# YaqiangCao/cLoops

Hardware: AMD Instinct MI355X
Metric: PETs clustered/sec (whole node) + wall-clock for mode-3 eps x minPts sweep (higher is better)
Workload: dtype int32; 1 GPU; synthetic-200M-23chr-mode3 (BASELINE.json configs[3]); variant=cDBSCAN2, pets=200000000, chromosomes=23, chained_cut=True, final_cut=3871, candidate_loops=3651369, parallelism=23 chromosomes LPT-sharded over 1 GPU(s)

## Files before the change

### cloops_amd/csrc/cl_chrom.h

```cpp
#pragma once
#include "cl_common.h"
#include "cl_table.h"
#include "cl_prim.h"
#include "cl_textout.h"

#define BIGTPB 1024
#define AGG_H 512
__device__ __forceinline__ int agg_slot(int* keys, int key)
{
    unsigned h = ((unsigned)key * 2654435761u) >> 23;
    for (int probe = 0; probe < 24; ++probe) {
        const int old = atomicCAS(&keys[h], -1, key);
        if (old == -1 || old == key) return (int)h;
        h = (h + 1) & (AGG_H - 1);
    }
    return -1;
}
#define FLAT_PER 4
struct Stats { int amin, amax, vmin, vmax, xmin, xmax, ymin, ymax; };
__device__ __forceinline__ int je_minus(const int* __restrict__ cstart, int j) { return cstart[j + 1] - cstart[j]; }
static inline int bits_for(unsigned v) { int b = 0; while (v) { ++b; v >>= 1; } return b; }


#define CL_FINE_KMAX 8
#define K7_BLOCKS 2048
#define K7_STEP_BLOCKS 256
#define K7_STEP_THREADS 1024
#define K7_LOGBINS 3840
__device__ __forceinline__ int k7_logbin(unsigned d)
{
    const int e = 31 - __clz((int)d);
    const unsigned m = e >= 7 ? ((d >> (e - 7)) & 127u) : ((d << (7 - e)) & 127u);
    return e * 128 + (int)m;
}
#define K7_FINE 2048
#define K7_XSHIFT 11.0
#define CAND_BLOCK 2048

struct K7Src {
    int sorted;
    int n; int M; int v0;
    const int* dM;
    const int* X; const int* Y; const int* labels;
    const int* sv; const int* slab;
    const int* dh;
};

struct K7Part { double sx[2]; double sxx[2]; long long n_all[2]; long long n_pos[2]; };

enum { HDR_K = 0, HDR_ERR = 1, HDR_M = 2, HDR_NCLUSTERS = 3, HDR_MAXLABEL = 4, HDR_TRUNC = 5, HDR_LABELLED = 6, HDR_WORDS = 16 };
enum { HDR_ERR_STRIP = 4 , HDR_ERR_COUNT = 8  };

struct RunRequest {
    int variant = CL_VARIANT_CDBSCAN1, eps = 0, minPts = 0, cut = 0;
    int32_t* labels_out = nullptr;
    int2* pairs_out = nullptr;
    long long pairs_cap = 0;
    void* mask_out = nullptr;
    long long mask_cap = 0;
    int step = -1;
    long long fine_lo = -1;
    int wx = 0, wy = 0;
};

struct cl_chrom {
    long long tmp_n = -1;
    DevBuf arena;
    int device = 0;
    hipStream_t stream = nullptr;
    bool own_stream = false;
    int64_t n = 0;
    int *d_x = nullptr, *d_y = nullptr;
    bool own_xy = false;
    Stats st{};
    DevBuf keys_in, keys_out, vals_in, vals_out, sort_tmp, scan_tmp;
    DevBuf qb_key, qb_val;
    int qindex_layout = -1;
    struct Fine {
        DevBuf q, sp, row, strip;
        DevBuf dead;
        int w = 0;
        int valid_w = 0, layout = -1;
        GridParams g;
        void invalidate() { valid_w = 0; layout = -1; }
    } fine;
    int sort_index_mode = 0;
    long long n_sorts = 0;
    DevBuf sv, sa, strip, cnt, parent, root, head, headidx, cellfirst, compkey, ncore, bsize, owner, state;
    DevBuf flag, rankscan, ulist, lo, hi, recs, counters, chainflag, chainhead, usize, b_cstart, b_ckey, b_nb, b_cx, b_cy, tile_s0;
    int* h_pinned = nullptr;
    struct StripPlan { int layout, eps, maxlen; };
    std::vector<StripPlan> plans;
    struct Held {
        int32_t* labels_out = nullptr;
        struct Extra {
            void* dst = nullptr;
            long long cap = 0;
            size_t fixed = 0; int per = 0;
            bool copy_empty = false;
            const char* refusal = nullptr;
        } extra;
        int n_strips = 0;
        bool band_timed = false;
        long long n_queried = 0;
        bool exported = false;
        bool step_valid = false;
        bool host_written = false;
        bool wait_done = false;
        long long fine_lo = -1;
        bool rows_valid = false;
        bool sorted_src = false;
        const int* k7_sv = nullptr;
        const int* k7_lcnt = nullptr;
        int k7_v0 = 0;
    };
    struct Run {
        u32* srow = nullptr;
        int *sv = nullptr, *sa = nullptr, *strip = nullptr, *tile = nullptr;
        int* cnt = nullptr;
        WordSrc ws{};
        int init_nclr = 0;
        int level = 0;
        const int* dM = nullptr;
        int m = 0;
        bool m_exact = false;
        bool rows = true;
        bool l4_make_base = false;
        bool l4_cut = false;
        bool l4_band = false;
        bool k2_make = false;
        const int* k_total = nullptr;
        bool hdr_packed = false;
        int kmax = 0;
        Held held;
    } run;
    struct Base {
        DevBuf q, sp, row, strip, tile, key;
        bool valid = false; int layout = -1, eps = 0;
        bool key_valid = false;
        int floor_q = 0;
        int rows = 0;
        long long pad_rows = -1;
        void invalidate() { valid = false; key_valid = false; floor_q = 0; }
    } base;
    bool sweep_planned = false;
    DevBuf sel_tmp;
    struct Counts {
        bool valid = false;
        bool cut_on_base = false;
        bool base_space = false;
        int layout = -1, eps = 0, thr = 0 , cap = 0;
        u32 tmask[4] = {0, 0, 0, 0};
        DevBuf cnt, pre, poff, dpre, D, blen;
        void invalidate() { valid = false; }
    } rc;
    bool reuse_counts = true;
    int count_floor = 0;
    u32 count_tmask[4] = {0, 0, 0, 0};
    DevBuf blk_tmp;
    DevBuf rootlist, cflag8;
    DevBuf l_mask, l_rank, l_blk, l_cstrip, l_wpos, l_wenc, l_dist, l_aux;
    DevBuf l_tab, l_fix;
    bool pairs_defer = false, pairs_copy_pending = false;
    bool fuse_chains = true;
    bool l_sup_dirty = false;
    GridParams dbg_g{}; int dbg_nm = 0;
    int traversal = 4;
    int last_k2_mode = 0;
    std::vector<long long> dcum;
    DevBuf dhist;
    long long n_neg = 0;
    bool reuse_layout = true;
    struct Slot {
        DevBuf labels, table;
        DevBuf slab;
        DevBuf pairs;
        DevBuf d_step;
        hipEvent_t ev_done = nullptr, ev_copied = nullptr;
        hipEvent_t ev[10]{};
        int* h_hdr = nullptr;
        char* h_step = nullptr;
        cl_box* h_boxes = nullptr;
        size_t h_boxes_cap = 0;
        bool pending = false;
        Held held;
    } slot[2];
    bool device_labels = true;
    bool export_table = true;
    struct Cand { DevBuf box, step, keep, out; long long n = 0, cap = 0; } cand;
    DevBuf hdr;
    DevBuf k7_cls, k7_parts;
    struct Kde {
        DevBuf ent, sorted, ctr, tmp, part;
        int run = -1;
        long long cap = 0, cnt[2] = {0, 0};
    } kde;
    struct Sig { DevBuf tx, ty, tmp, sorttmp, m, win, out; bool ready = false; int cut = 0; } sig;
    struct Fp { DevBuf small, keys, sorted, tmp, pairs; } fp;
    struct Anchor { DevBuf s, e, dir, mask, wsum; } an;
    struct Agg {
        DevBuf kin, vin, sx, sy, tmp, m, cx, cy, lkin, lkout, lvin, order, ltmp, sum, stats, mats;
        bool ready = false; int cut = 0, kept = 0;
    } ag;
    struct Track {
        DevBuf tcnt, toff, row, keys, sorted, tmp, ids, names;
        TextOut txt;
        struct State {
            bool built = false, ids = false;
            int kind = 0, la = 0, lb = 0, gbits = 0;
            long long cut = 0, ext = 0;
        } st;
    } tk;
    struct Cov {
        DevBuf kin, key, tmp, dcur, dprev, xr, flag, scan, ctr, start, end, depth, name;
// ... 279 lines not shown
```

### cloops_amd/csrc/cloops_hip.hip

```cpp
#include <map>
#include <mutex>
#include "cl_chrom.h"
#include "cl_band.h"

thread_local std::string g_err;



extern "C" const char* cl_last_error(void) { return g_err.c_str(); }
extern "C" int cl_version(void) { return CL_VERSION_NUM; }

extern "C" void* cl_host_alloc(int64_t bytes)
{
    void* p = nullptr;
    if (bytes <= 0) return nullptr;
    if (hipHostMalloc(&p, (size_t)bytes, hipHostMallocDefault) != hipSuccess) { fail(CL_ERR_HIP, "hipHostMalloc"); return nullptr; }
    return p;
}
extern "C" void cl_host_free(void* p) { if (p) (void)hipHostFree(p); }

static std::mutex g_pair_mu;
static std::map<hipStream_t, hipStream_t> g_copy_of;
extern "C" void* cl_stream_create(int device)
{
// ... 2786 lines not shown
__global__ void k_pack_header(int* __restrict__ hdr, const int* __restrict__ rankscan_total, const int* __restrict__ counters,
                              const int* __restrict__ d_M)
{
    if (threadIdx.x == 0 && blockIdx.x == 0) {
        hdr[HDR_K] = rankscan_total[0];
        hdr[HDR_ERR] = counters[CTR_OVERFLOW];
        hdr[HDR_M] = d_M[0];
        hdr[HDR_NCLUSTERS] = 0;
        hdr[HDR_MAXLABEL] = -1;
        hdr[HDR_TRUNC] = 0;
    }
}

__global__ void k_export_table(int* __restrict__ hdr, Table t, cl_box* __restrict__ host_rows, int cap)
{
    const int K = hdr[HDR_K];
    const bool store = cap >= 0;
    const int lim = store ? min(K, cap) : K;
    int nc = 0, ml = -1;
    for (int k = blockIdx.x * blockDim.x + threadIdx.x; k < lim; k += gridDim.x * blockDim.x) {
        if (store) {
            cl_box b = t.get(k);
            if (b.count > 0) { ++nc; ml = k; } else { b.min_x = b.max_x = b.min_y = b.max_y = 0; }
            host_rows[k] = b;
        } else if (t.count[k] > 0) { ++nc; ml = k; }
    }
    for (int o = 32; o > 0; o >>= 1) { nc += __shfl_down(nc, o); ml = max(ml, __shfl_down(ml, o)); }
    if ((threadIdx.x & 63) == 0) {
        if (nc) atomicAdd(&hdr[HDR_NCLUSTERS], nc);
        if (ml >= 0) atomicMax(&hdr[HDR_MAXLABEL], ml);
    }
    if (blockIdx.x == 0 && threadIdx.x == 0 && store && K > cap) hdr[HDR_TRUNC] = 1;
}

Table make_table_slot(cl_chrom* c, int slot)
{
    Table t;
    int* base = c->slot[slot].table.as<int>();
    const size_t stride = (size_t)c->n + 1;
    t.count = base; t.minx = base + stride; t.maxx = base + 2 * stride; t.miny = base + 3 * stride; t.maxy = base + 4 * stride;
    return t;
}
Table make_table(cl_chrom* c) { return make_table_slot(c, c->cur); }

const int* k7_hist_for(cl_chrom* c, int cut)
{
    return (cut > 0 && cut < DCUM_BINS && c->n_neg == 0 && !c->dcum.empty() && c->dhist.p) ? c->dhist.as<int>() : (const int*)nullptr;
}

K7Src k7_src(cl_chrom* c, const cl_chrom::Held& r, cl_chrom::Slot& sl, int cut, int M, const int* dM)
{
    K7Src s{};
    s.sorted = r.sorted_src ? (r.k7_lcnt ? 2 : 1) : 0; s.n = (int)c->n; s.M = M; s.v0 = r.k7_v0; s.dM = r.k7_lcnt ? r.k7_lcnt : dM;
    s.X = c->d_x; s.Y = c->d_y; s.labels = sl.labels.as<int>(); s.sv = r.k7_sv; s.slab = sl.slab.as<int>();
    s.dh = k7_hist_for(c, cut);
    return s;
}

int finish_enqueue(cl_chrom* c, const RunRequest& req, int n_strips, const int* d_M)
{
    const int n = (int)c->n;
    int32_t* const labels_out = req.labels_out;
    cl_chrom::Slot& sl = c->slot[c->cur];
    cl_chrom::Held& held = c->run.held;
    int* dh = c->hdr.as<int>() + HDR_WORDS * c->cur;
    if (sl.h_boxes_cap == 0 && c->export_table && req.step < 0) {
        const size_t cap = (size_t)n / 16 + 65536;
        HIP_TRY(hipHostMalloc((void**)&sl.h_boxes, cap * sizeof(cl_box), hipHostMallocDefault));
        sl.h_boxes_cap = cap;
    }
    if (!c->run.hdr_packed)
        hipLaunchKernelGGL(k_pack_header, dim3(1), dim3(64), 0, c->stream, dh, c->run.k_total ? c->run.k_total : c->rankscan.as<int>() + n, c->counters.as<int>(), d_M);
    const bool exported = c->export_table && req.step < 0;
    if (req.step < 0)
        hipLaunchKernelGGL(k_export_table, dim3(256), dim3(TPB), 0, c->stream, dh, make_table(c), sl.h_boxes,
                           exported ? (int)std::min<size_t>(sl.h_boxes_cap, 0x7fffffff) : -1);
    held.exported = exported;
    if (req.step >= 0) {
        int rc;
        if ((rc = c->k7_cls.ensure((size_t)n + 16))) return rc;
        const int kmax = std::max(1, std::min(c->run.kmax, n));
        if ((rc = ensure_cand_capacity(c, c->cand.n + kmax))) return rc;
        const size_t out_bytes = 16 + sizeof(K7Part) + K7_LOGBINS * 8 + K7_FINE * 8;
        if ((rc = sl.d_step.ensure(out_bytes + K7_BLOCKS * sizeof(K7Part)))) return rc;
        const int nb = nblocks(kmax, CAND_BLOCK);
        if ((rc = c->sel_tmp.ensure((size_t)nb * 12 + 64))) return rc;
        int* bcount = c->sel_tmp.as<int>();
        Table t = make_table(c);
        signed char* cls = c->k7_cls.as<signed char>();
        char* ds = (char*)sl.d_step.p;
        unsigned long long* lh = (unsigned long long*)(ds + 16 + sizeof(K7Part));
        hipLaunchKernelGGL(k_step_classify_count, dim3(nb), dim3(256), 0, c->stream, (const int*)dh, t, cls, bcount, nb,
                           lh, K7_LOGBINS + K7_FINE);
        hipLaunchKernelGGL(k_cand_append, dim3(nb), dim3(256), 0, c->stream, (const int*)dh, cls, t, (const int*)nullptr, (const int*)bcount,
                           (int)c->cand.n, req.step, (int)std::min<long long>(c->cand.cap, INT_MAX), c->cand.box.as<int4>(), c->cand.step.as<int>());
        K7Part* parts = (K7Part*)(ds + out_bytes);
        const K7Src src = k7_src(c, held, sl, req.cut, 0, d_M);
        int k7b = K7_STEP_BLOCKS;
#ifdef CLOOPS_DEVEL
        int k7t = K7_STEP_THREADS;
        { const char* e = getenv("CLOOPS_K7B"); if (e) k7b = std::max(1, std::min(atoi(e), K7_BLOCKS)); e = getenv("CLOOPS_K7T"); if (e) k7t = atoi(e); }
#else
        const int k7t = K7_STEP_THREADS;
#endif
        if (!SKIP(16)) hipLaunchKernelGGL(k7_summary, dim3(k7b), dim3(k7t), 0, c->stream, src, req.cut, cls, parts, lh,
                           (unsigned)req.fine_lo, req.fine_lo >= 0 ? lh + K7_LOGBINS : (unsigned long long*)nullptr);
        static_assert((16 + sizeof(K7Part)) % 8 == 0, "step output in 8-byte words");
// ... 383 lines not shown
                       pmax32, c->parent.as<int>());
    if (level == 0 && !SKIP(4)) hipLaunchKernelGGL(k_flatten, dim3(nblocks(nm, BIGTPB * FLAT_PER)), dim3(BIGTPB), 0, c->stream, g, strip, (const int*)nullptr, (const int*)c->chainflag.as<int>(),
           c->parent.as<int>(), srow, c->head.as<int>(), c->cellfirst.as<int>(),
           c->root.as<int>(), c->compkey.as<int>(), c->ncore.as<int>(), c->rootlist.as<int>(), counters);
    int* rootlist = c->rootlist.as<int>();
    ev_record(c, 4);
    int* clist = c->chainflag.as<int>();
    if (level >= 2) { if ((rc = lists_border(c, g, nm, L))) return rc; }
    else if (wide == 0) {
        const int nt_b = nblocks(std::max(1, c->run.m), 1024);
        if (!SKIP(1)) hipLaunchKernelGGL((k_border<1024, 128, TPB>), dim3(tile_grid(nt_b)), dim3(TPB), 0, c->stream, g, nt_b, sv, sa, strip, c->root.as<int>(),
                           c->compkey.as<int>(), c->ncore.as<int>(), srow, c->owner.as<int>(), c->bsize.as<int>(), c->usize.as<int>(), ws, clist, counters);
    } else
    TILE_LAUNCH_H((wide >= 2 && wide <= 4) ? 512 : (wide >= 5 ? 256 : 128), k_border, g, ntiles, sv, sa, strip, c->root.as<int>(), c->compkey.as<int>(),
                       c->ncore.as<int>(), srow, c->owner.as<int>(), c->bsize.as<int>(), c->usize.as<int>(), ws, clist, counters);
    if (variant == CL_VARIANT_CDBSCAN2) {
        const int rec_cap = n;
        hipLaunchKernelGGL(k_mark_uncertain_l, dim3(512), dim3(TPB), 0, c->stream, g, rootlist, c->ncore.as<int>(), c->bsize.as<int>(), c->state.as<int>(),
                           c->ulist.as<int>(), counters);
        if (level >= 2) { if ((rc = lists_emit_records(c, g, nm, L))) return rc; }
        else if (!SKIP(128)) hipLaunchKernelGGL(k_emit_records, dim3(2048), dim3(TPB), 0, c->stream, g, sv, sa, strip, c->root.as<int>(),
                           c->compkey.as<int>(), c->state.as<int>(), c->owner.as<int>(), c->recs.as<Rec>(), rec_cap, counters,
                           (const int*)clist, ws);
        hipLaunchKernelGGL(k_resolve_release, dim3(1), dim3(1024), 0, c->stream, minPts, c->ncore.as<int>(), c->usize.as<int>(), c->state.as<int>(),
                           c->ulist.as<int>(), c->recs.as<Rec>(), c->lo.as<int>(), c->hi.as<int>(), counters);
    }
    ev_record(c, 5);
    hipLaunchKernelGGL(k_rank_bits_l, dim3(512), dim3(TPB), 0, c->stream, g, rootlist, counters, c->compkey.as<int>(), c->state.as<int>(), c->flag.as<unsigned>(),
                       variant == CL_VARIANT_CDBSCAN2 ? (const Rec*)c->recs.as<Rec>() : (const Rec*)nullptr, c->owner.as<int>());
    const int nblkw = nblocks(nw, 1024);
    if ((rc = c->blk_tmp.ensure(((size_t)nblkw + 2) * 8))) return rc;
    int* wbsum = c->blk_tmp.as<int>();
    int* wboff = wbsum + nblkw + 1;
    hipLaunchKernelGGL(k_rank_scan, dim3(nblkw), dim3(256), 0, c->stream, nw, (const unsigned*)c->flag.as<unsigned>(), c->rankscan.as<int>(), wbsum, wboff,
                       counters + CTR_TICKET_B);
    c->run.k_total = wboff + nblkw;
    Table t = make_table(c);
    hipLaunchKernelGGL(k_root_labels_bits_l, dim3(512), dim3(TPB), 0, c->stream, g, rootlist, counters, c->compkey.as<int>(), c->ncore.as<int>(), c->bsize.as<int>(),
                       c->state.as<int>(), c->flag.as<unsigned>(), (const int*)c->rankscan.as<int>(), (const int*)wboff, c->chainhead.as<int>(), t, nblkw,
                       c->hdr.as<int>() + HDR_WORDS * c->cur, c->run.dM ? c->run.dM : (const int*)(strip + g.S));
    c->run.hdr_packed = true;
    if (level >= 3) {
        int* const labelled = c->hdr.as<int>() + HDR_WORDS * c->cur + HDR_LABELLED;
        if (req.pairs_out) {
            held.extra = {req.pairs_out, req.pairs_cap, 0, 8, false, "cl_cluster_pairs_async: the run labelled more PETs than capacity_pairs (n always suffices)"};
            if ((rc = c->slot[c->cur].pairs.ensure((size_t)std::max<long long>(req.pairs_cap, 1) * 8))) return rc;
        }
        if ((rc = lists_final(c, req, g, nm, L, rows, labelled))) return rc;
        if (req.mask_out) {
            held.extra = {req.mask_out, req.mask_cap, (size_t)((n + 63) / 64) * 8, 4, true, "cl_cluster_rowmask_async: the run labelled more PETs than capacity_labels (n always suffices)"};
            if ((rc = lists_rowmask(c, req, labelled))) return rc;
        }
        held.k7_lcnt = L.lcnt; held.k7_sv = c->l_dist.as<int>();
    } else {
        if (req.mask_out) return fail(CL_ERR_ARG, "cl_cluster_rowmask_async: this run did not take the list form");
        if (level == 2 && (rc = lists_scatter_owner(c, nm, L))) return rc;
        if (!SKIP(8)) hipLaunchKernelGGL(k_final_labels, dim3(nblocks(nm, BIGTPB * FINAL_CHUNKS)), dim3(BIGTPB), 0, c->stream, g, strip, sv, sa, srow,
                       level == 2 ? c->l_aux.as<int>() : c->owner.as<int>(),
                       c->chainhead.as<int>(), rows ? c->slot[c->cur].labels.as<int>() : (int*)nullptr, c->slot[c->cur].slab.as<int>(), t);
    }
    HIP_TRY(hipGetLastError());
    rc = finish_enqueue(c, req, g.S + 2, c->run.dM ? c->run.dM : strip + g.S);
    guard.armed = rc != CL_OK;
    return rc;
}


extern "C" int cl_get_boxes(cl_chrom* c, cl_box* boxes_out)
{
    if (!c) return fail(CL_ERR_ARG, "null chromosome handle");
    if (!c->have_result) return fail(CL_ERR_ARG, "cl_get_boxes: no clustering result available");
    const int K = c->last_K;
    if (K <= 0) return CL_OK;
    if (!boxes_out) return fail(CL_ERR_ARG, "boxes_out is null");
    if (c->last_slot >= 0 && !c->slot[c->last_slot].held.exported) return fail(CL_ERR_ARG, "cl_get_boxes: the run was made with the table export switched off");
    memcpy(boxes_out, c->slot[c->last_slot].h_boxes, (size_t)K * sizeof(cl_box));
    return CL_OK;
}

extern "C" int64_t cl_last_n_in(const cl_chrom* c)
{
    if (!c || !c->have_result || c->last_slot < 0) return 0;
    return c->slot[c->last_slot].h_hdr[HDR_M];
}

extern "C" const cl_box* cl_boxes_host(const cl_chrom* c)
{
    if (!c || !c->have_result || c->last_slot < 0 || c->last_K <= 0 || !c->slot[c->last_slot].held.exported) return nullptr;
    return c->slot[c->last_slot].h_boxes;
}
```

### cloops_amd/csrc/k_lists.hip

```cpp
#include "cl_chrom.h"

#ifdef CLOOPS_DEVEL
#define L_ABL(bit) (g.dbg2 & (bit))
#else
#define L_ABL(bit) 0
#endif
#ifdef CLOOPS_DEVEL
__device__ unsigned long long g_lstat[32];
__device__ __forceinline__ void lstat_add(int slot, int v)
{
    int t = v;
    for (int o = 32; o > 0; o >>= 1) t += __shfl_down(t, o);
    if ((threadIdx.x & 63) == 0 && t) atomicAdd(&g_lstat[slot], (unsigned long long)t);
}
extern "C" void cl_debug_lstats(unsigned long long* out)
{
    (void)hipDeviceSynchronize();
    (void)hipMemcpyFromSymbol(out, HIP_SYMBOL(g_lstat), sizeof(g_lstat));
    unsigned long long z[32] = {0};
    (void)hipMemcpyToSymbol(HIP_SYMBOL(g_lstat), z, sizeof(z));
}
#define LSTAT_ON (g.dbg2 & (1 << 30))
#define LSTAT(slot, v) do { if (LSTAT_ON) lstat_add((slot), (v)); } while (0)
#else
// ... 1566 lines not shown
            auto more = [&](int w, int q, int p) {
                return w == 0 ? ((p >= pbeg) & (q >= qlo)) : w == 1 ? ((p < pend) & (q <= qhi)) : w == 2 ? ((p < pbeg) & (q <= qhi)) : ((p < pend2) & (q <= qhi));
            };
            auto acc = [&](int w, int p) { return w == 2 ? p >= plo : (w == 3 ? p <= phi : true); };
            auto round = [&](int w, bool on, bool in, int2 p, int r) {
                const bool ok = on && in && more(w, p.x, p.y);
                const int rv = (ok && acc(w, p.y)) ? r : -1;
                unsigned pending = (unsigned)(__ballot(rv >= 0) >> gsh) & 0xffffu;
                while (__any(pending != 0u)) {
                    const int R = __shfl(rv, gsh + (pending ? __ffs((int)pending) - 1 : 0));
                    const unsigned same = (unsigned)(__ballot(pending != 0u && rv == R) >> gsh) & 0xffffu;
                    if (pending) { see(R); pending &= ~same; }
                }
                return on && ((unsigned)(__ballot(ok) >> gsh) & 0xffffu) == 0xffffu;
            };
            int2 p0[4]; int r0[4]; bool in0[4];
#pragma unroll
            for (int w = 0; w < 4; ++w) {
                const int j = w == 0 ? start[w] - gl : start[w] + gl;
                in0[w] = act && j >= 0 && j < C;
                p0[w] = in0[w] ? cpair[j] : make_int2(0, 0); r0[w] = in0[w] ? croot[j] : -1;
            }
#pragma unroll
            for (int w = 0; w < 4; ++w) {
                bool on = round(w, act, in0[w], p0[w], r0[w]);
                for (int rnd = 1; __any(on); ++rnd) {
                    const int j = w == 0 ? start[w] - gl - EG * rnd : start[w] + gl + EG * rnd;
                    const bool in = on && j >= 0 && j < C;
                    on = round(w, on, in, in ? cpair[j] : make_int2(0, 0), in ? croot[j] : -1);
                }
            }
            if (act && gl == 0) {
                if (overflow) atomicExch(&counters[CTR_OVERFLOW], 1);
                if (any_u) {
                    const int idx = atomicAdd(&counters[CTR_NREC], 1);
                    if (idx >= rec_cap) atomicExch(&counters[CTR_OVERFLOW], 2);
                    else {
                        Rec rec; rec.pt = h;
                        for (int q = 0; q < 4; ++q) rec.r[q] = rr[q];
                        recs[idx] = rec;
                    }
                }
            }
        }
    }
}

#ifndef LF_TPB
#define LF_TPB BIGTPB
#endif
#ifndef LF_CHUNKS
#define LF_CHUNKS 2
#endif
__global__ void __launch_bounds__(LF_TPB)
k_final_lists(GridParams g, const int* __restrict__ lcnt, const int2* __restrict__ cpair, const int* __restrict__ cpos,
              const int* __restrict__ croot, const int2* __restrict__ wpair, const int* __restrict__ wpos,
              const int* __restrict__ wowner, const int* __restrict__ rlabel, const u32* __restrict__ srow,
              int* __restrict__ labels, int* __restrict__ llab, int* __restrict__ ldist, Table t,
              int2* __restrict__ pairs , int pairs_cap,
              int* __restrict__ pair_count)
{
    __shared__ TableLds h;
    table_lds_init(h);
    const int C = lcnt[0], L = C + lcnt[1];
    int idx[LF_CHUNKS], own[LF_CHUNKS], lab[LF_CHUNKS], x[LF_CHUNKS], y[LF_CHUNKS], pos[LF_CHUNKS];
    int2 pr[LF_CHUNKS];
#pragma unroll
    for (int ch = 0; ch < LF_CHUNKS; ++ch) {
        idx[ch] = (blockIdx.x * LF_CHUNKS + ch) * LF_TPB + threadIdx.x;
        const int k = idx[ch];
        own[ch] = -1; pos[ch] = 0; pr[ch] = make_int2(0, 0);
        if (k < C) { own[ch] = croot[k]; pr[ch] = cpair[k]; pos[ch] = (labels || pairs) ? cpos[k] : 0; }
        else if (k < L) { own[ch] = owner_root(wowner[k - C]); pr[ch] = wpair[k - C]; pos[ch] = (labels || pairs) ? wpos[k - C] : 0; }
    }
#pragma unroll
    for (int ch = 0; ch < LF_CHUNKS; ++ch) lab[ch] = own[ch] >= 0 ? rlabel[own[ch]] : -1;
#pragma unroll
    for (int ch = 0; ch < LF_CHUNKS; ++ch) {
        const int k = idx[ch];
        x[ch] = 0; y[ch] = 0;
        if (k < L) {
            llab[k] = lab[ch];
            ldist[k] = pr[ch].x;
            if (lab[ch] >= 0) {
                if (labels) labels[srow[pos[ch]]] = lab[ch];
                const int spv = pr[ch].y;
                const int pp = ((spv >> g.rbits) + g.s0) * g.eps + (spv & (g.peps - 1)) + g.A0, qq = pr[ch].x + g.V0;
                const int a = g.swap ? qq : pp, v = g.swap ? pp : qq;
                x[ch] = (v - a) / 2; y[ch] = (v + a) / 2;
            }
        }
    }
    if (pairs) {
        __shared__ int l_pc[LF_CHUNKS * (LF_TPB / 64)];
        __shared__ int l_pbase;
        const int lane = threadIdx.x & 63, wv = threadIdx.x >> 6;
        unsigned long long bals[LF_CHUNKS];
#pragma unroll
        for (int ch = 0; ch < LF_CHUNKS; ++ch) {
            bals[ch] = __ballot(lab[ch] >= 0);
            if (lane == 0) l_pc[ch * (LF_TPB / 64) + wv] = __popcll(bals[ch]);
        }
        __syncthreads();
        if (threadIdx.x == 0) {
            int tot = 0;
            for (int k = 0; k < LF_CHUNKS * (LF_TPB / 64); ++k) { const int v = l_pc[k]; l_pc[k] = tot; tot += v; }
            l_pbase = tot ? atomicAdd(pair_count, tot) : 0;
        }
        __syncthreads();
#pragma unroll
        for (int ch = 0; ch < LF_CHUNKS; ++ch) {
            if (lab[ch] < 0) continue;
            const int at = l_pbase + l_pc[ch * (LF_TPB / 64) + wv] + lane_rank(bals[ch]);
            if (at < pairs_cap) pairs[at] = make_int2((int)srow[pos[ch]], lab[ch]);
        }
    }
    if (L_ABL(1 << 10)) return;
#pragma unroll
    for (int ch = 0; ch < LF_CHUNKS; ++ch) table_accumulate(t, h, lab[ch], x[ch], y[ch]);
    if (L_ABL(1 << 9)) return;
    table_flush(t, h);
}

struct ListBufs {
    unsigned long long *cmask, *wmask, *hmask;
    int *cgloc, *wgloc, *cgrank, *wgrank;
    int *bsum, *sup, *lcnt;
    int nsup2;
};
static int list_bufs(cl_chrom* c, const GridParams& g, int nm, ListBufs* b)
{
    const size_t n = (size_t)c->n;
    const size_t ngrp_cap = n / 64 + LG + 4;
    const size_t nblk_cap = n / LT + 4;
    int rc;
    if ((rc = c->l_mask.ensure(3 * ngrp_cap * 8)) || (rc = c->l_rank.ensure(4 * ngrp_cap * 4)) ||
        (rc = c->l_blk.ensure((2 * (nblk_cap + 1) + 2 * (nblk_cap / 16 + 4) + 16) * 4)) || (rc = c->l_cstrip.ensure(((size_t)g.S + 4) * 4)) ||
        (rc = c->l_wpos.ensure(n * 4)) || (rc = c->l_wenc.ensure(n * 4)) || (rc = c->l_dist.ensure(n * 4)) ||
        (c->traversal < 3 && (rc = c->l_aux.ensure(n * 4)))) return rc;
    b->cmask = c->l_mask.as<unsigned long long>(); b->wmask = b->cmask + ngrp_cap; b->hmask = b->wmask + ngrp_cap;
    b->cgloc = c->l_rank.as<int>(); b->wgloc = b->cgloc + ngrp_cap; b->cgrank = b->wgloc + ngrp_cap; b->wgrank = b->cgrank + ngrp_cap;
    const int nblk = nblocks(nm, LT);
    const size_t nsup_cap = nblk_cap / 16 + 4;
    if (c->l_blk.fresh) {
        HIP_TRY(hipMemsetAsync(c->l_blk.p, 0, c->l_blk.bytes, c->stream));
        c->l_blk.fresh = false;
    }
    b->lcnt = c->l_blk.as<int>();
    b->sup = b->lcnt + 8;
    b->bsum = b->sup + 2 * nsup_cap;
    b->nsup2 = 2 * ((nblk + 63) / 64 + 1);
    return CL_OK;
}

static void launch_classify(cl_chrom* c, const GridParams& g, int nblk, const ListBufs& b)
{
#define LA_ARGS g, (const int*)c->run.sv, (const int*)c->run.sa, (const int*)c->run.strip, c->run.ws, (const u32*)c->run.srow, b.cmask, b.wmask, b.hmask, b.cgloc, b.wgloc, b.bsum, b.sup, c->cellfirst.as<int>()
    if (g.variant == CL_VARIANT_CDBSCAN2) hipLaunchKernelGGL(k_classify<true>, dim3(nblk), dim3(256), 0, c->stream, LA_ARGS);
    else hipLaunchKernelGGL(k_classify<false>, dim3(nblk), dim3(256), 0, c->stream, LA_ARGS);
#undef LA_ARGS
}
static void launch_make_lists(cl_chrom* c, const GridParams& g, int nblk, const ListBufs& b, const ListRun& L)
{
#define LM_ARGS g, (const int*)c->run.sv, (const int*)c->run.sa, (const int*)c->run.strip, c->run.ws, (const u32*)c->run.srow, (const unsigned long long*)b.cmask,                   \
                (const unsigned long long*)b.wmask, (const unsigned long long*)b.hmask, (const int*)b.cgloc, (const int*)b.wgloc, (const int*)b.bsum, (const int*)b.sup,  \
                (const int*)c->cellfirst.as<int>(), b.cgrank, b.wgrank, L.cpair, L.cpos, L.ckey, L.wpair, L.wpos, L.wenc, b.lcnt
    if (g.variant == CL_VARIANT_CDBSCAN2) hipLaunchKernelGGL(k_make_lists<true>, dim3(nblk), dim3(256), 0, c->stream, LM_ARGS);
    else hipLaunchKernelGGL(k_make_lists<false>, dim3(nblk), dim3(256), 0, c->stream, LM_ARGS);
#undef LM_ARGS
}
static void list_views(cl_chrom* c, const ListBufs& b, ListRun* L)
{
    L->lcnt = b.lcnt; L->cmask = b.cmask; L->wmask = b.wmask; L->cgrank = b.cgrank; L->wgrank = b.wgrank;
    L->cpair = c->keys_in.as<int2>(); L->wpair = c->keys_out.as<int2>();
    L->cpos = c->head.as<int>(); L->ckey = c->hi.as<int>();
    L->wpos = c->l_wpos.as<int>(); L->wenc = c->l_wenc.as<int>(); L->cstrip = c->l_cstrip.as<int>();
}

static inline void fuse_knob(cl_chrom* c)
{
#ifdef CLOOPS_DEVEL
    const char* e = getenv("CLOOPS_FUSE");
    if (e) c->fuse_chains = atoi(e) != 0;
#else
    (void)c;
#endif
}

int lists_build(cl_chrom* c, const GridParams& g, int nm, ListRun* out)
{
    ListBufs b;
    int rc = list_bufs(c, g, nm, &b);
// ... 155 lines not shown
    bool queued = true;
#ifdef CLOOPS_DEVEL
    { const char* e = getenv("CLOOPS_BCAP"); if (e) kcap = atoi(e); queued = kcap > 0; e = getenv("CLOOPS_BQG"); if (e) bqg = atoi(e); }
#endif
    const int nt = nblocks(std::max(1, L.npos), (g.variant == CL_VARIANT_CDBSCAN1 || !queued) ? BNT : BNQ);
#define LB_ARGS g, nt, L.npos, L.lcnt, L.cmask, L.cgrank, L.wgrank, (const int2*)L.cpair, (const int*)croot_of(c), (const int*)c->cellfirst.as<int>(),    \
                (const int*)L.ckey, (const int*)L.cstrip, (const int2*)L.wpair, (const int*)L.wpos, (const int*)L.wenc, (const int*)c->compkey.as<int>(),                    \
                (const int*)c->ncore.as<int>(), c->owner.as<int>(), c->bsize.as<int>(), c->usize.as<int>(), c->chainflag.as<int>() ,  \
                c->counters.as<int>()
    if (g.variant == CL_VARIANT_CDBSCAN1) hipLaunchKernelGGL((k_border_w<BNT, BHC, true>), dim3(ltile_grid(nt)), dim3(256), 0, c->stream, LB_ARGS);
#ifdef CLOOPS_DEVEL
    else if (!queued) hipLaunchKernelGGL((k_border_w<BNT, BHC, false>), dim3(ltile_grid(nt)), dim3(256), 0, c->stream, LB_ARGS);
#endif
#define LBQ_ARGS g, nt, L.npos, kcap, L.lcnt, L.cmask, L.cgrank, L.wgrank, (const int2*)L.cpair, (const int*)croot_of(c), (const int*)c->cellfirst.as<int>(),           \
                 (const int*)L.cstrip, (const int2*)L.wpair, (const int*)L.wpos, (const int*)L.wenc, (const int*)c->compkey.as<int>(), (const int*)c->ncore.as<int>(),        \
                 c->owner.as<int>(), c->bsize.as<int>(), c->usize.as<int>(), c->chainflag.as<int>(), c->counters.as<int>()
#ifdef CLOOPS_DEVEL
    else if (bqg == 8) hipLaunchKernelGGL((k_border_q<BNQ, BHQ, 8>), dim3(ltile_grid(nt)), dim3(256), 0, c->stream, LBQ_ARGS);
    else if (bqg == 32) hipLaunchKernelGGL((k_border_q<BNQ, BHQ, 32>), dim3(ltile_grid(nt)), dim3(256), 0, c->stream, LBQ_ARGS);
#endif
    else hipLaunchKernelGGL((k_border_q<BNQ, BHQ, 16>), dim3(ltile_grid(nt)), dim3(256), 0, c->stream, LBQ_ARGS);
    (void)bqg;
#undef LBQ_ARGS
#undef LB_ARGS
    HIP_TRY(hipGetLastError());
    return CL_OK;
}

int lists_emit_records(cl_chrom* c, const GridParams& g, int nm, const ListRun& L)
{
    (void)nm;
    hipLaunchKernelGGL(k_emit_records_w, dim3(2048), dim3(TPB), 0, c->stream, g, L.lcnt, L.cmask, L.cgrank, (const int2*)L.cpair, (const int*)croot_of(c),
                       (const int*)L.cstrip, (const int2*)L.wpair, (const int*)L.wpos, (const int*)L.wenc, (const int*)c->compkey.as<int>(),
                       (const int*)c->state.as<int>(), (const int*)c->owner.as<int>(), c->recs.as<Rec>(), (int)c->n, c->counters.as<int>(),
                       (const int*)c->chainflag.as<int>());
    HIP_TRY(hipGetLastError());
    return CL_OK;
}

int lists_scatter_owner(cl_chrom* c, int nm, const ListRun& L)
{
    int* opos = c->l_aux.as<int>();
    HIP_TRY(hipMemsetAsync(opos, 0xFF, (size_t)nm * 4, c->stream));
    LAUNCH(k_scatter_by_pos, nm, L.lcnt, (const int*)L.cpos, (const int*)croot_of(c), opos);
    LAUNCH(k_scatter_by_pos, nm, L.lcnt + 1, (const int*)L.wpos, (const int*)c->owner.as<int>(), opos);
    return CL_OK;
}

int lists_final(cl_chrom* c, const RunRequest& req, const GridParams& g, int nm, const ListRun& L, bool rows, int* pair_count)
{
    cl_chrom::Slot& sl = c->slot[c->cur];
    hipLaunchKernelGGL(k_final_lists, dim3(nblocks(nm, LF_TPB * LF_CHUNKS)), dim3(LF_TPB), 0, c->stream, g, L.lcnt, (const int2*)L.cpair, (const int*)L.cpos,
                       (const int*)croot_of(c), (const int2*)L.wpair, (const int*)L.wpos, (const int*)c->owner.as<int>(), (const int*)c->chainhead.as<int>(),
                       (const u32*)c->run.srow, (rows && !req.pairs_out) ? sl.labels.as<int>() : (int*)nullptr, sl.slab.as<int>(), c->l_dist.as<int>(), make_table(c),
                       req.pairs_out ? sl.pairs.as<int2>() : (int2*)nullptr, (int)std::min<long long>(req.pairs_cap, INT_MAX), pair_count);
    HIP_TRY(hipGetLastError());
    return CL_OK;
}

#define RM_T 2048
__global__ void __launch_bounds__(256)
k_rowmask_count(int n, const int* __restrict__ labels, unsigned long long* __restrict__ mask, int* __restrict__ tsum,
                unsigned long long* __restrict__ sup)
{
    __shared__ int l_c[4];
    const int t0 = (int)blockIdx.x * RM_T;
    const int lane = threadIdx.x & 63, wv = threadIdx.x >> 6;
    int lab[8];
#pragma unroll
    for (int u = 0; u < 8; ++u) { const int r = t0 + u * 256 + (int)threadIdx.x; lab[u] = r < n ? labels[r] : -1; }
    int cnt = 0;
#pragma unroll
    for (int u = 0; u < 8; ++u) {
        const unsigned long long bal = __ballot(lab[u] >= 0);
        if (lane == 0 && t0 + u * 256 + wv * 64 < n) mask[(t0 >> 6) + u * 4 + wv] = bal;
        cnt += __popcll(bal);
    }
    if (lane == 0) l_c[wv] = cnt;
    __syncthreads();
    if (threadIdx.x == 0) {
        const int tot = l_c[0] + l_c[1] + l_c[2] + l_c[3];
        tsum[blockIdx.x] = tot;
        if (tot) atomicAdd(&sup[blockIdx.x >> 4], (unsigned long long)tot);
    }
}
__global__ void __launch_bounds__(256)
k_rowmask_write(int n, const int* __restrict__ labels, const unsigned long long* __restrict__ mask, const int* __restrict__ tsum,
                const unsigned long long* __restrict__ sup, int* __restrict__ out, long long cap, int* __restrict__ total)
{
    __shared__ long long l_red[4];
    __shared__ int l_goff[RM_T / 64];
    const int blk = (int)blockIdx.x, t0 = blk * RM_T;
    const int lane = threadIdx.x & 63, wv = threadIdx.x >> 6;
    int lab[8];
#pragma unroll
    for (int u = 0; u < 8; ++u) { const int r = t0 + u * 256 + (int)threadIdx.x; lab[u] = r < n ? labels[r] : -1; }
    long long pc = 0;
    const int sb = blk >> 4;
    for (int k = threadIdx.x; k < sb; k += 256) pc += (long long)sup[k];
    if (threadIdx.x < 16) { const int k = sb * 16 + (int)threadIdx.x; if (k < blk) pc += tsum[k]; }
#pragma unroll
    for (int o = 32; o > 0; o >>= 1) pc += __shfl_down(pc, o);
    if (lane == 0) l_red[wv] = pc;
    if (threadIdx.x < 64) {
        const int k = lane & 31;
        const int gi = (t0 >> 6) + k;
        const int v = (lane < 32 && (long long)gi * 64 < n) ? __popcll(mask[gi]) : 0;
// ... 114 lines not shown
```

### cloops_amd/csrc/k_sweep.hip

```cpp
#include "cl_chrom.h"
#include "cl_log2_tab.h"

__global__ void k7_classify(const int* __restrict__ hdr, Table t, signed char* __restrict__ cls)
{
    const int K = hdr[HDR_K];
    int k = blockIdx.x * blockDim.x + threadIdx.x;
    if (k >= K) return;
    const cl_box b = t.get(k);
    signed char c = -1;
    if (b.count > 0 && b.min_x != b.max_x && b.min_y != b.max_y)
        c = (b.max_x < b.min_y) ? 0 : 1;
    cls[k] = c;
}


#ifndef K7_LIBM_LOG2
#define K7_LIBM_LOG2 0
#endif
__device__ __forceinline__ double k7_log2(unsigned d, const double* __restrict__ rcp, const double* __restrict__ lg)
{
    const int e = 31 - __clz((int)d);
    const unsigned k = ((d << (31 - e)) >> 24) & 127u;
    const double m = __hiloint2double((int)(0x3ff00000u | (((d << (31 - e)) & 0x7fffffffu) >> 11)), (int)(d << (31 - e) << 21));
    const double r = fma(m, rcp[k], -1.0);
    double p = -0.24044917348149393;
    p = fma(p, r, 0.28853900817779268);
    p = fma(p, r, -0.36067376022224085);
    p = fma(p, r, 0.48089834696298783);
    p = fma(p, r, -0.72134752044448170);
    p = fma(p, r, 1.4426950408889634);
    return ((double)e + lg[k]) + p * r;
}
template <typename F>
__device__ __forceinline__ void k7_for_each(const K7Src& s, int cut, const signed char* __restrict__ cls, F&& f)
{
    if (s.sorted) {
        const int M = s.sorted == 2 ? s.dM[0] + s.dM[1] : (s.dM ? s.dM[0] : s.M);
        const int per = (M + gridDim.x - 1) / gridDim.x;
        const int i0 = blockIdx.x * per, i1 = min(M, i0 + per);
        int i = i0 + threadIdx.x;
        const int bd = blockDim.x;
        for (; i + 3 * bd < i1; i += 4 * bd) {
            int lab[4], d[4], g[4];
#pragma unroll
            for (int k = 0; k < 4; ++k) { lab[k] = s.slab[i + k * bd]; d[k] = s.sv[i + k * bd] + s.v0; }
#pragma unroll
            for (int k = 0; k < 4; ++k) g[k] = lab[k] >= 0 ? (int)cls[lab[k]] : -1;
#pragma unroll
            for (int k = 0; k < 4; ++k) if (g[k] >= 0) f(g[k], d[k] < 0 ? -d[k] : d[k], 1);
        }
        for (; i < i1; i += bd) {
            const int lab = s.slab[i];
            const int g = lab >= 0 ? (int)cls[lab] : -1;
            const int d = s.sv[i] + s.v0;
            if (g >= 0) f(g, d < 0 ? -d : d, 1);
        }
        if (cut > 0 && s.dh) {
            for (int d = blockIdx.x * blockDim.x + threadIdx.x; d < cut; d += gridDim.x * blockDim.x) {
                const int w = s.dh[d];
                if (w) f(1, d, w);
            }
        } else if (cut > 0) {
            const int perr = (s.n + gridDim.x - 1) / gridDim.x;
            const int r0 = blockIdx.x * perr, r1 = min(s.n, r0 + perr);
            for (int r = r0 + threadIdx.x; r < r1; r += blockDim.x) {
                const int d = s.Y[r] - s.X[r];
                if (d < cut) f(1, d < 0 ? -d : d, 1);
            }
        }
    } else {
        const int perr = (s.n + gridDim.x - 1) / gridDim.x;
        const int r0 = blockIdx.x * perr, r1 = min(s.n, r0 + perr);
        for (int r = r0 + threadIdx.x; r < r1; r += blockDim.x) {
            const int d = s.Y[r] - s.X[r];
            int g = 1;
            if (!(cut > 0 && d < cut)) { const int lab = s.labels[r]; g = lab >= 0 ? (int)cls[lab] : -1; }
            if (g >= 0) f(g, d < 0 ? -d : d, 1);
        }
    }
}


__device__ __forceinline__ void k7_reduce_block(const K7Part* __restrict__ parts, int nparts, K7Part* __restrict__ out,
                                                const int* __restrict__ bcount , int nb, long long* __restrict__ totals,
                                                double (*sd)[256], long long (*sn)[256])
{
    const int tid = threadIdx.x;
    double a[4] = {0, 0, 0, 0}; long long c[6] = {0, 0, 0, 0, 0, 0};
    for (int k = tid; k < nparts; k += 256) {
        const K7Part p = parts[k];
        a[0] += p.sx[0]; a[1] += p.sx[1]; a[2] += p.sxx[0]; a[3] += p.sxx[1];
        c[0] += p.n_all[0]; c[1] += p.n_all[1]; c[2] += p.n_pos[0]; c[3] += p.n_pos[1];
    }
    if (bcount) for (int k = tid; k < nb; k += 256) { c[4] += bcount[k]; c[5] += bcount[nb + k]; }
    for (int q = 0; q < 4; ++q) { sd[q][tid] = a[q]; sn[q][tid] = c[q]; }
    __syncthreads();
    for (int o = 128; o > 0; o >>= 1) {
        if (tid < o) for (int q = 0; q < 4; ++q) { sd[q][tid] += sd[q][tid + o]; sn[q][tid] += sn[q][tid + o]; }
        __syncthreads();
    }
    if (tid == 0) {
        K7Part p;
        p.sx[0] = sd[0][0]; p.sx[1] = sd[1][0]; p.sxx[0] = sd[2][0]; p.sxx[1] = sd[3][0];
        p.n_all[0] = sn[0][0]; p.n_all[1] = sn[1][0]; p.n_pos[0] = sn[2][0]; p.n_pos[1] = sn[3][0];
        *out = p;
    }
    if (bcount) {
        __syncthreads();
        sn[0][tid] = c[4]; sn[1][tid] = c[5];
// ... 785 lines not shown
```

Baseline: 16.40 billion PETs/s.

## Compact labelled list items per segment and skip dead slots in sweep

```diff
diff --git a/cloops_amd/csrc/cl_chrom.h b/cloops_amd/csrc/cl_chrom.h
--- a/cloops_amd/csrc/cl_chrom.h
+++ b/cloops_amd/csrc/cl_chrom.h
@@ -5,6 +5,9 @@
 #include "cl_textout.h"
 
 #define BIGTPB 1024
+#define LSEG_BITS 11
+#define LSEG (1 << LSEG_BITS)
+static_assert(LSEG % 64 == 0, "a segment is whole waves of list items");
 #define AGG_H 512
 __device__ __forceinline__ int agg_slot(int* keys, int key)
 {
@@ -43,6 +46,7 @@
     const int* dM;
     const int* X; const int* Y; const int* labels;
     const int* sv; const int* slab;
+    const int* seg_cnt;
     const int* dh;
 };
 
@@ -112,6 +116,7 @@
         bool sorted_src = false;
         const int* k7_sv = nullptr;
         const int* k7_lcnt = nullptr;
+        const int* k7_seg = nullptr;
         int k7_v0 = 0;
     };
     struct Run {
@@ -160,6 +165,7 @@
     DevBuf blk_tmp;
     DevBuf rootlist, cflag8;
     DevBuf l_mask, l_rank, l_blk, l_cstrip, l_wpos, l_wenc, l_dist, l_aux;
+    DevBuf l_seg;
     DevBuf l_tab, l_fix;
     bool pairs_defer = false, pairs_copy_pending = false;
     bool fuse_chains = true;
diff --git a/cloops_amd/csrc/cloops_hip.hip b/cloops_amd/csrc/cloops_hip.hip
--- a/cloops_amd/csrc/cloops_hip.hip
+++ b/cloops_amd/csrc/cloops_hip.hip
@@ -2862,7 +2862,7 @@
 {
     K7Src s{};
     s.sorted = r.sorted_src ? (r.k7_lcnt ? 2 : 1) : 0; s.n = (int)c->n; s.M = M; s.v0 = r.k7_v0; s.dM = r.k7_lcnt ? r.k7_lcnt : dM;
-    s.X = c->d_x; s.Y = c->d_y; s.labels = sl.labels.as<int>(); s.sv = r.k7_sv; s.slab = sl.slab.as<int>();
+    s.X = c->d_x; s.Y = c->d_y; s.labels = sl.labels.as<int>(); s.sv = r.k7_sv; s.slab = sl.slab.as<int>(); s.seg_cnt = r.k7_seg;
     s.dh = k7_hist_for(c, cut);
     return s;
 }
@@ -3352,6 +3352,7 @@
             if ((rc = lists_rowmask(c, req, labelled))) return rc;
         }
         held.k7_lcnt = L.lcnt; held.k7_sv = c->l_dist.as<int>();
+        held.k7_seg = c->l_seg.as<int>();
     } else {
         if (req.mask_out) return fail(CL_ERR_ARG, "cl_cluster_rowmask_async: this run did not take the list form");
         if (level == 2 && (rc = lists_scatter_owner(c, nm, L))) return rc;
diff --git a/cloops_amd/csrc/k_lists.hip b/cloops_amd/csrc/k_lists.hip
--- a/cloops_amd/csrc/k_lists.hip
+++ b/cloops_amd/csrc/k_lists.hip
@@ -1642,17 +1642,23 @@
 #ifndef LF_CHUNKS
 #define LF_CHUNKS 2
 #endif
+#define LF_WAVES (LF_CHUNKS * (LF_TPB / 64))
+static_assert(LF_CHUNKS * LF_TPB == LSEG, "one workgroup of k_final_lists makes one segment of the label / distance list");
+static_assert(LF_WAVES <= 64, "one wave scans the wave counts of a segment");
 __global__ void __launch_bounds__(LF_TPB)
 k_final_lists(GridParams g, const int* __restrict__ lcnt, const int2* __restrict__ cpair, const int* __restrict__ cpos,
               const int* __restrict__ croot, const int2* __restrict__ wpair, const int* __restrict__ wpos,
               const int* __restrict__ wowner, const int* __restrict__ rlabel, const u32* __restrict__ srow,
-              int* __restrict__ labels, int* __restrict__ llab, int* __restrict__ ldist, Table t,
+              int* __restrict__ labels, int* __restrict__ llab, int* __restrict__ ldist, int* __restrict__ seg_cnt, Table t,
               int2* __restrict__ pairs , int pairs_cap,
               int* __restrict__ pair_count)
 {
     __shared__ TableLds h;
+    __shared__ int l_pc[LF_WAVES];
+    __shared__ int l_pbase;
     table_lds_init(h);
     const int C = lcnt[0], L = C + lcnt[1];
+    const bool want_pos = labels || pairs;
     int idx[LF_CHUNKS], own[LF_CHUNKS], lab[LF_CHUNKS], x[LF_CHUNKS], y[LF_CHUNKS], pos[LF_CHUNKS];
     int2 pr[LF_CHUNKS];
 #pragma unroll
@@ -1660,49 +1666,45 @@
         idx[ch] = (blockIdx.x * LF_CHUNKS + ch) * LF_TPB + threadIdx.x;
         const int k = idx[ch];
         own[ch] = -1; pos[ch] = 0; pr[ch] = make_int2(0, 0);
-        if (k < C) { own[ch] = croot[k]; pr[ch] = cpair[k]; pos[ch] = (labels || pairs) ? cpos[k] : 0; }
-        else if (k < L) { own[ch] = owner_root(wowner[k - C]); pr[ch] = wpair[k - C]; pos[ch] = (labels || pairs) ? wpos[k - C] : 0; }
+        if (k < C) { own[ch] = croot[k]; pr[ch] = cpair[k]; pos[ch] = want_pos ? cpos[k] : 0; }
+        else if (k < L) { own[ch] = owner_root(wowner[k - C]); pr[ch] = wpair[k - C]; pos[ch] = want_pos ? wpos[k - C] : 0; }
     }
 #pragma unroll
     for (int ch = 0; ch < LF_CHUNKS; ++ch) lab[ch] = own[ch] >= 0 ? rlabel[own[ch]] : -1;
+    const int lane = threadIdx.x & 63, wv = threadIdx.x >> 6;
+    unsigned long long bals[LF_CHUNKS];
 #pragma unroll
     for (int ch = 0; ch < LF_CHUNKS; ++ch) {
-        const int k = idx[ch];
+        bals[ch] = __ballot(lab[ch] >= 0);
+        if (lane == 0) l_pc[ch * (LF_TPB / 64) + wv] = __popcll(bals[ch]);
+    }
+    __syncthreads();
+    if (threadIdx.x < 64) {
+        const int v = lane < LF_WAVES ? l_pc[lane] : 0;
+        int incl = v;
+#pragma unroll
+        for (int o = 1; o < LF_WAVES; o <<= 1) { const int up = __shfl_up(incl, o); if (lane >= o) incl += up; }
+        if (lane < LF_WAVES) l_pc[lane] = incl - v;
+        if (lane == LF_WAVES - 1) {
+            seg_cnt[blockIdx.x] = incl;
+            if (pairs) l_pbase = incl ? atomicAdd(pair_count, incl) : 0;
+        }
+    }
+    __syncthreads();
+    const int seg0 = blockIdx.x * LSEG;
+#pragma unroll
+    for (int ch = 0; ch < LF_CHUNKS; ++ch) {
         x[ch] = 0; y[ch] = 0;
-        if (k < L) {
-            llab[k] = lab[ch];
-            ldist[k] = pr[ch].x;
-            if (lab[ch] >= 0) {
-                if (labels) labels[srow[pos[ch]]] = lab[ch];
-                const int spv = pr[ch].y;
-                const int pp = ((spv >> g.rbits) + g.s0) * g.eps + (spv & (g.peps - 1)) + g.A0, qq = pr[ch].x + g.V0;
-                const int a = g.swap ? qq : pp, v = g.swap ? pp : qq;
-                x[ch] = (v - a) / 2; y[ch] = (v + a) / 2;
-            }
-        }
-    }
-    if (pairs) {
-        __shared__ int l_pc[LF_CHUNKS * (LF_TPB / 64)];
-        __shared__ int l_pbase;
-        const int lane = threadIdx.x & 63, wv = threadIdx.x >> 6;
-        unsigned long long bals[LF_CHUNKS];
-#pragma unroll
-        for (int ch = 0; ch < LF_CHUNKS; ++ch) {
-            bals[ch] = __ballot(lab[ch] >= 0);
-            if (lane == 0) l_pc[ch * (LF_TPB / 64) + wv] = __popcll(bals[ch]);
-        }
-        __syncthreads();
-        if (threadIdx.x == 0) {
-            int tot = 0;
-            for (int k = 0; k < LF_CHUNKS * (LF_TPB / 64); ++k) { const int v = l_pc[k]; l_pc[k] = tot; tot += v; }
-            l_pbase = tot ? atomicAdd(pair_count, tot) : 0;
-        }
-        __syncthreads();
-#pragma unroll
-        for (int ch = 0; ch < LF_CHUNKS; ++ch) {
-            if (lab[ch] < 0) continue;
-            const int at = l_pbase + l_pc[ch * (LF_TPB / 64) + wv] + lane_rank(bals[ch]);
-            if (at < pairs_cap) pairs[at] = make_int2((int)srow[pos[ch]], lab[ch]);
+        if (lab[ch] >= 0) {
+            const int at = l_pc[ch * (LF_TPB / 64) + wv] + lane_rank(bals[ch]);
+            llab[seg0 + at] = lab[ch];
+            ldist[seg0 + at] = pr[ch].x;
+            if (labels) labels[srow[pos[ch]]] = lab[ch];
+            if (pairs && l_pbase + at < pairs_cap) pairs[l_pbase + at] = make_int2((int)srow[pos[ch]], lab[ch]);
+            const int spv = pr[ch].y;
+            const int pp = ((spv >> g.rbits) + g.s0) * g.eps + (spv & (g.peps - 1)) + g.A0, qq = pr[ch].x + g.V0;
+            const int a = g.swap ? qq : pp, v = g.swap ? pp : qq;
+            x[ch] = (v - a) / 2; y[ch] = (v + a) / 2;
         }
     }
     if (L_ABL(1 << 10)) return;
@@ -1727,7 +1729,7 @@
     if ((rc = c->l_mask.ensure(3 * ngrp_cap * 8)) || (rc = c->l_rank.ensure(4 * ngrp_cap * 4)) ||
         (rc = c->l_blk.ensure((2 * (nblk_cap + 1) + 2 * (nblk_cap / 16 + 4) + 16) * 4)) || (rc = c->l_cstrip.ensure(((size_t)g.S + 4) * 4)) ||
         (rc = c->l_wpos.ensure(n * 4)) || (rc = c->l_wenc.ensure(n * 4)) || (rc = c->l_dist.ensure(n * 4)) ||
-        (c->traversal < 3 && (rc = c->l_aux.ensure(n * 4)))) return rc;
+        (rc = c->l_seg.ensure((n / LSEG + 2) * 4)) || (c->traversal < 3 && (rc = c->l_aux.ensure(n * 4)))) return rc;
     b->cmask = c->l_mask.as<unsigned long long>(); b->wmask = b->cmask + ngrp_cap; b->hmask = b->wmask + ngrp_cap;
     b->cgloc = c->l_rank.as<int>(); b->wgloc = b->cgloc + ngrp_cap; b->cgrank = b->wgloc + ngrp_cap; b->wgrank = b->cgrank + ngrp_cap;
     const int nblk = nblocks(nm, LT);
@@ -1989,7 +1991,7 @@
     cl_chrom::Slot& sl = c->slot[c->cur];
     hipLaunchKernelGGL(k_final_lists, dim3(nblocks(nm, LF_TPB * LF_CHUNKS)), dim3(LF_TPB), 0, c->stream, g, L.lcnt, (const int2*)L.cpair, (const int*)L.cpos,
                        (const int*)croot_of(c), (const int2*)L.wpair, (const int*)L.wpos, (const int*)c->owner.as<int>(), (const int*)c->chainhead.as<int>(),
-                       (const u32*)c->run.srow, (rows && !req.pairs_out) ? sl.labels.as<int>() : (int*)nullptr, sl.slab.as<int>(), c->l_dist.as<int>(), make_table(c),
+                       (const u32*)c->run.srow, (rows && !req.pairs_out) ? sl.labels.as<int>() : (int*)nullptr, sl.slab.as<int>(), c->l_dist.as<int>(), c->l_seg.as<int>(), make_table(c),
                        req.pairs_out ? sl.pairs.as<int2>() : (int2*)nullptr, (int)std::min<long long>(req.pairs_cap, INT_MAX), pair_count);
     HIP_TRY(hipGetLastError());
     return CL_OK;
diff --git a/cloops_amd/csrc/k_sweep.hip b/cloops_amd/csrc/k_sweep.hip
--- a/cloops_amd/csrc/k_sweep.hip
+++ b/cloops_amd/csrc/k_sweep.hip
@@ -34,8 +34,43 @@
 template <typename F>
 __device__ __forceinline__ void k7_for_each(const K7Src& s, int cut, const signed char* __restrict__ cls, F&& f)
 {
-    if (s.sorted) {
-        const int M = s.sorted == 2 ? s.dM[0] + s.dM[1] : (s.dM ? s.dM[0] : s.M);
+    if (s.sorted == 2) {
+        const int M = s.dM[0] + s.dM[1];
+        const int per = (M + gridDim.x - 1) / gridDim.x;
+        const int i0 = blockIdx.x * per, i1 = min(M, i0 + per);
+        int i = i0 + threadIdx.x;
+        const int bd = blockDim.x;
+        int sc[4];
+#pragma unroll
+        for (int k = 0; k < 4; ++k) { const int j = i + k * bd; sc[k] = j < i1 ? s.seg_cnt[j >> LSEG_BITS] : 0; }
+        for (; i + 3 * bd < i1; i += 4 * bd) {
+            int lab[4], d[4], g[4], nsc[4];
+            bool live[4];
+#pragma unroll
+            for (int k = 0; k < 4; ++k) {
+                const int j = i + k * bd, jn = j + 4 * bd;
+                live[k] = (j & (LSEG - 1)) < sc[k];
+                nsc[k] = jn < i1 ? s.seg_cnt[jn >> LSEG_BITS] : 0;
+                lab[k] = 0; d[k] = 0;
+                if (live[k]) { lab[k] = s.slab[j]; d[k] = s.sv[j] + s.v0; }
+            }
+#pragma unroll
+            for (int k = 0; k < 4; ++k) g[k] = live[k] ? (int)cls[lab[k]] : -1;
+#pragma unroll
+            for (int k = 0; k < 4; ++k) if (g[k] >= 0) f(g[k], d[k] < 0 ? -d[k] : d[k], 1);
+#pragma unroll
+            for (int k = 0; k < 4; ++k) sc[k] = nsc[k];
+        }
+#pragma unroll
+        for (int k = 0; k < 3; ++k) {
+            const int j = i + k * bd;
+            if (j >= i1 || (j & (LSEG - 1)) >= sc[k]) continue;
+            const int g = (int)cls[s.slab[j]];
+            const int d = s.sv[j] + s.v0;
+            if (g >= 0) f(g, d < 0 ? -d : d, 1);
+        }
+    } else if (s.sorted) {
+        const int M = s.dM ? s.dM[0] : s.M;
         const int per = (M + gridDim.x - 1) / gridDim.x;
         const int i0 = blockIdx.x * per, i1 = min(M, i0 + per);
         int i = i0 + threadIdx.x;
@@ -55,6 +90,8 @@
             const int d = s.sv[i] + s.v0;
             if (g >= 0) f(g, d < 0 ? -d : d, 1);
         }
+    }
+    if (s.sorted) {
         if (cut > 0 && s.dh) {
             for (int d = blockIdx.x * blockDim.x + threadIdx.x; d < cut; d += gridDim.x * blockDim.x) {
                 const int w = s.dh[d];
```

After: 16.37 billion PETs/s. Within noise of the previous version (-0.2%).
